# hpcaitech/SkyComputing

Hardware: AMD Instinct MI355X
Metric: sec_per_iter_bert160_mnli_bsz32 (lower is better)
Workload: dtype bf16; 1 GPU; model=bert-160L-H1024-A16, global_batch=32, seq_len=128, parallelism=pp1, microbatches=1, schedule=gpipe, allocate=even, num_pipeline_layers=483, hipgraph=True

## Files before the change

skycomputing_amd/ops/hip/attention.hip:

```cpp

#include "attn_common.h"

#define K_OFF 0
#define VT_OFF 0
#define P_OFF (16 * 1024)
#define ATT_LDS_BYTES (48 * 1024)

template <bool HAS_MASK, bool SAVE_ML, bool PROBS_MODE, bool TRV = false>
__global__ __launch_bounds__(256, 2) void attn_fwd_kernel(
    const ushort_t* __restrict__ qkv, const ushort_t* __restrict__ mask,
    ushort_t* __restrict__ out, float* __restrict__ m_io,
    float* __restrict__ l_io, ushort_t* __restrict__ p_out,
    ushort_t* __restrict__ pd_out, int B, int S, int h, float scale,
    float keep, uint64_t salt, const unsigned long long* __restrict__ state) {
  extern __shared__ __attribute__((aligned(16))) char lds[];
  const int tid = threadIdx.x;
  const int l = tid & 63;
  const int w = tid >> 6;
  const int bh = blockIdx.x;
  const int b = bh / h;
  const int hh = bh % h;
  const int ts = 3 * h * ATT_D;
  const int NT = (S + 15) / 16;
  const uint64_t seed = rng_seed(salt, state);
// ... 123 lines not shown
  att_zero(oacc[1]);

  __syncthreads();
  if (TRV) {
    att_glds_rows(vbase, ts, 0, 128, true, S, lds, VT_OFF, tid);
    asm volatile("s_waitcnt vmcnt(0)" ::: "memory");
  } else {
    if (S < ATT_SMAX) {
      for (int u = tid; u < (16 * 1024) / 16; u += 256)
        *(ushort8_t*)lds_at(lds, VT_OFF + u * 16) = (ushort8_t)(ushort_t)0;
      __syncthreads();
    }
    for (int u = tid; u < S * 8; u += 256) {
      const int tok = u >> 3;
      const int c16 = u & 7;
      ushort8_t v = *(const ushort8_t*)(vbase + (size_t)tok * ts + c16 * 8);
#pragma unroll
      for (int jj = 0; jj < 8; ++jj) {
        const int j = (jj + tok) & 7;
        const int c = c16 * 8 + j;
        *(ushort_t*)lds_at(lds, swz(VT_OFF + c * 256 + tok * 2, c, 15)) = v[j];
      }
    }
  }
  __syncthreads();

  for (int qi = 0; qi < 2; ++qi) {
    if ((qt0 + qi) * 16 >= S) break;
#pragma unroll
    for (int ks = 0; ks < 4; ++ks) {
      if (ks * 32 >= S) break;
      const int rl = qi * 16 + lm;
      bf16x8 ap = *(const bf16x8*)lds_at(
          lds, swz(P_OFF + w * 8192 + rl * 256 + (ks * 32 + lg * 8) * 2, rl, 15));
#pragma unroll
      for (int dvt = 0; dvt < 4; ++dvt) {
        bf16x8 bv;
        if (TRV) {
          bv = abf_tr_rows64(lds, VT_OFF, ks * 32 + lg * 8, dvt * 4, lm);
        } else {
          const int dv = dvt * 16 + lm;
          bv = *(const bf16x8*)lds_at(
              lds, swz(VT_OFF + dv * 256 + (ks * 32 + lg * 8) * 2, dv, 15));
        }
        oacc[qi][dvt] =
            __builtin_amdgcn_mfma_f32_16x16x32_bf16(ap, bv, oacc[qi][dvt], 0, 0, 0);
      }
    }
  }
  ushort_t* obase = out + ((size_t)b * S * h + hh) * ATT_D;
#pragma unroll
  for (int qi = 0; qi < 2; ++qi)
    att_store_rows16(obase, h * ATT_D, oacc[qi], (qt0 + qi) * 16, S, lm, lg);
}

template <int DT>
__global__ __launch_bounds__(256) void pack3_kernel(
    const void* __restrict__ s0, const void* __restrict__ s1,
    const void* __restrict__ s2, void* __restrict__ dst, int64_t B,
    int64_t S, int64_t h, int64_t d8) {
  const int64_t n = B * h * S * d8;
  for (int64_t u = (int64_t)blockIdx.x * 256 + threadIdx.x; u < n;
       u += (int64_t)gridDim.x * 256) {
    int64_t t = u;
    const int64_t di = t % d8; t /= d8;
    const int64_t tok = t % S; t /= S;
    const int64_t hh = t % h;
    const int64_t b = t / h;
    const int64_t src_off = u;
    const int64_t dst_base = (((b * S + tok) * 3) * h + hh) * d8 + di;
    float v[8];
    Vec8<DT>::load(s0, src_off, v);
    Vec8<DT>::store(dst, dst_base, v);
    Vec8<DT>::load(s1, src_off, v);
    Vec8<DT>::store(dst, dst_base + h * d8, v);
    Vec8<DT>::load(s2, src_off, v);
    Vec8<DT>::store(dst, dst_base + 2 * h * d8, v);
  }
}

SKY_EXPORT int sky_pack3(uint64_t stream, uint64_t s0, uint64_t s1,
                         uint64_t s2, uint64_t dst, int64_t B, int64_t S,
                         int64_t h, int64_t d, int dt) {
  if (d % 8 != 0) return (int)hipErrorInvalidValue;
  const int64_t n = B * h * S * (d / 8);
  unsigned grid = (unsigned)((n + 255) / 256);
  if (grid > 2048u) grid = 2048u;
  hipStream_t s = (hipStream_t)stream;
  if (dt == DT_F32)
    hipLaunchKernelGGL((pack3_kernel<DT_F32>), dim3(grid), dim3(256), 0, s,
                       (const void*)s0, (const void*)s1, (const void*)s2,
                       (void*)dst, B, S, h, d / 8);
  else
    hipLaunchKernelGGL((pack3_kernel<DT_BF16>), dim3(grid), dim3(256), 0, s,
                       (const void*)s0, (const void*)s1, (const void*)s2,
                       (void*)dst, B, S, h, d / 8);
  LAUNCH_CHECK();
  return 0;
}

static int attn_launch(uint64_t stream, uint64_t qkv, uint64_t mask,
                       uint64_t out, uint64_t m, uint64_t lsum, uint64_t p,
                       uint64_t pd, int64_t B, int64_t S, int64_t h,
                       int64_t d, float scale, float keep, uint64_t salt,
                       uint64_t state, bool probs_mode) {
  if (d != ATT_D || S > ATT_SMAX) return (int)hipErrorInvalidValue;
  hipStream_t s = (hipStream_t)stream;
  dim3 grid((unsigned)(B * h));
  size_t lds_bytes = ATT_LDS_BYTES;
  bool hm = mask != 0;
  const char* trve = getenv("SKY_ATTN_TRV");
  const bool trv = !(trve && trve[0] == '0');
#define ATT(SML, PM, TRV)                                                     \
  ATT_LAUNCH_HM(hm, (attn_fwd_kernel<HM, SML, PM, TRV>), grid, lds_bytes, s,  \
                (const ushort_t*)qkv, (const ushort_t*)mask, (ushort_t*)out,  \
                (float*)m, (float*)lsum, (ushort_t*)p, (ushort_t*)pd, (int)B, \
                (int)S, (int)h, scale, keep, salt,                            \
                (const unsigned long long*)state)
  if (probs_mode) { if (trv) ATT(false, true, true); else ATT(false, true, false); }
  else            { if (trv) ATT(true, false, true); else ATT(true, false, false); }
#undef ATT
  LAUNCH_CHECK();
  return 0;
}

SKY_EXPORT int sky_attn_fwd(uint64_t stream, uint64_t qkv, uint64_t mask,
                            uint64_t out, uint64_t m, uint64_t lsum,
                            int64_t B, int64_t S, int64_t h, int64_t d,
                            float scale, float keep, uint64_t salt,
                            uint64_t state) {
  return attn_launch(stream, qkv, mask, out, m, lsum, 0, 0, B, S, h, d,
                     scale, keep, salt, state, false);
}

SKY_EXPORT int sky_attn_probs(uint64_t stream, uint64_t qkv, uint64_t mask,
                              uint64_t m, uint64_t lsum, uint64_t p,
                              uint64_t pd, int64_t B, int64_t S, int64_t h,
                              int64_t d, float scale, float keep,
                              uint64_t salt, uint64_t state) {
  return attn_launch(stream, qkv, mask, 0, m, lsum, p, pd, B, S, h, d, scale,
                     keep, salt, state, true);
}
```

skycomputing_amd/ops/hip/attention_bwd.hip:

```cpp

#include "attn_common.h"

template <bool HAS_MASK, bool DBIAS>
__global__ __launch_bounds__(256, 3) void attn_bwd1s_kernel(
    const ushort_t* __restrict__ qkv, const ushort_t* __restrict__ dout,
    const ushort_t* __restrict__ mask, const float* __restrict__ m_io,
    const float* __restrict__ l_io, ushort_t* __restrict__ pdT,
    ushort_t* __restrict__ dsT, ushort_t* __restrict__ dqkv, int B, int S,
    int h, float scale, float keep, uint64_t salt,
    const unsigned long long* __restrict__ state, float* __restrict__ dbscr) {
  extern __shared__ __attribute__((aligned(16))) char lds[];
  const int tid = threadIdx.x;
  const int l = tid & 63;
  const int w = tid >> 6;
  const int lm = l & 15;
  const int lg = l >> 4;
  const int QB = (S + 63) / 64;
  const int bh = blockIdx.x / QB;
  const int qb = blockIdx.x % QB;
  const int b = bh / h;
  const int hh = bh % h;
  const int ts = 3 * h * ATT_D;
  const int NT = (S + 15) / 16;
  const uint64_t seed = rng_seed(salt, state);
// ... 389 lines not shown
      att_store_rows16(dq, ts, qacc, qtok_base, S, lm, lg);
    }

#pragma unroll
    for (int ks2 = 0; ks2 < 2; ++ks2) {
      const int q0t = ks2 * 32 + lg * 8;
      bf16x8 apd[2], ads[2];
#pragma unroll
      for (int ki = 0; ki < 2; ++ki) {
        const int kt = 2 * w + ki;
        apd[ki] = abf_tr_rows128(lds, ABF_PD, q0t, kt * 4, lm);
        ads[ki] = abf_tr_rows128(lds, ABF_DS, q0t, kt * 4, lm);
      }
#pragma unroll
      for (int ct = 0; ct < 4; ++ct) {
        bf16x8 bq = abf_tr_rows64(lds, ABF_Q, pass * 64 + q0t, ct * 4, lm);
        bf16x8 bdo = abf_tr_rows64(lds, ABF_DO, pass * 64 + q0t, ct * 4, lm);
#pragma unroll
        for (int ki = 0; ki < 2; ++ki) {
          vacc[ki][ct] = __builtin_amdgcn_mfma_f32_16x16x32_bf16(apd[ki], bdo, vacc[ki][ct], 0, 0, 0);
          kacc[ki][ct] = __builtin_amdgcn_mfma_f32_16x16x32_bf16(ads[ki], bq, kacc[ki][ct], 0, 0, 0);
        }
      }
    }
    __syncthreads();
  }

  ushort_t* dk = dqkv + (size_t)b * S * ts + (size_t)(h + hh) * ATT_D;
  ushort_t* dv = dqkv + (size_t)b * S * ts + (size_t)(2 * h + hh) * ATT_D;
#pragma unroll
  for (int ki = 0; ki < 2; ++ki)
    att_store_rows16x2(dk, dv, ts, kacc[ki], vacc[ki], (2 * w + ki) * 16, S,
                       lm, lg);
}

SKY_EXPORT int sky_attn_bwd_fused(uint64_t stream, uint64_t qkv,
                                  uint64_t dout, uint64_t mask, uint64_t m,
                                  uint64_t lsum, uint64_t dqkv, int64_t B,
                                  int64_t S, int64_t h, int64_t d,
                                  float scale, float keep, uint64_t salt,
                                  uint64_t state) {
  if (d != ATT_D || S > ATT_SMAX) return (int)hipErrorInvalidValue;
  hipStream_t s = (hipStream_t)stream;
  dim3 grid((unsigned)(B * h));
  ATT_LAUNCH_HM(mask != 0, (attn_bwd_fused_kernel<HM>), grid, ABF_LDS, s,
                (const ushort_t*)qkv, (const ushort_t*)dout,
                (const ushort_t*)mask, (const float*)m, (const float*)lsum,
                (ushort_t*)dqkv, (int)B, (int)S, (int)h, scale, keep, salt,
                (const unsigned long long*)state);
  LAUNCH_CHECK();
  return 0;
}

template <bool DBIAS>
static void launch_attn_bwd_pair(hipStream_t s, uint64_t qkv, uint64_t dout,
                                 uint64_t mask, uint64_t m, uint64_t lsum,
                                 uint64_t pdT, uint64_t dsT, uint64_t dqkv,
                                 int64_t B, int64_t S, int64_t h, float scale,
                                 float keep, uint64_t salt, uint64_t state,
                                 float* dbscr) {
  dim3 grid((unsigned)(B * h * ((S + 63) / 64)));
  ATT_LAUNCH_HM(mask != 0, (attn_bwd1s_kernel<HM, DBIAS>), grid, 48 * 1024, s,
                (const ushort_t*)qkv, (const ushort_t*)dout,
                (const ushort_t*)mask, (const float*)m, (const float*)lsum,
                (ushort_t*)pdT, (ushort_t*)dsT, (ushort_t*)dqkv, (int)B,
                (int)S, (int)h, scale, keep, salt,
                (const unsigned long long*)state, dbscr);
  hipLaunchKernelGGL(attn_bwd2_kernel<DBIAS>, dim3((unsigned)(B * h)),
                     dim3(256), (DBIAS ? 34 : 32) * 1024, s,
                     (const ushort_t*)qkv, (const ushort_t*)dout,
                     (const ushort_t*)pdT, (const ushort_t*)dsT,
                     (ushort_t*)dqkv, (int)B, (int)S, (int)h, dbscr);
}

SKY_EXPORT int sky_attn_bwd(uint64_t stream, uint64_t qkv, uint64_t dout,
                            uint64_t mask, uint64_t m, uint64_t lsum,
                            uint64_t pdT, uint64_t dsT, uint64_t dqkv,
                            int64_t B, int64_t S, int64_t h, int64_t d,
                            float scale, float keep, uint64_t salt,
                            uint64_t state) {
  if (d != ATT_D || S > ATT_SMAX) return (int)hipErrorInvalidValue;
  launch_attn_bwd_pair<false>((hipStream_t)stream, qkv, dout, mask, m, lsum,
                              pdT, dsT, dqkv, B, S, h, scale, keep, salt,
                              state, nullptr);
  LAUNCH_CHECK();
  return 0;
}

static int attn_bwd_dbias_impl(uint64_t stream, uint64_t qkv, uint64_t dout,
                               uint64_t mask, uint64_t m, uint64_t lsum,
                               uint64_t pdT, uint64_t dsT, uint64_t dqkv,
                               int64_t B, int64_t S, int64_t h, int64_t d,
                               float scale, float keep, uint64_t salt,
                               uint64_t state, uint64_t scratch,
                               uint64_t dbias, int dbias_dt,
                               SkyFinishJob* job) {
  if (d != ATT_D || S > ATT_SMAX || scratch == 0 || dbias == 0)
    return (int)hipErrorInvalidValue;
  hipStream_t s = (hipStream_t)stream;
  launch_attn_bwd_pair<true>(s, qkv, dout, mask, m, lsum, pdT, dsT, dqkv, B, S,
                             h, scale, keep, salt, state, (float*)scratch);
  const int64_t cols = 3 * h * ATT_D, nslabs = B * ((S + 63) / 64);
  if (job)
    sky_finish_job_set(job, scratch, dbias, 0, 0, nslabs, cols, 1, dbias_dt);
  else
    sky_launch_colsum_final(s, (const float*)scratch, (void*)dbias, cols,
                            nslabs, dbias_dt);
  LAUNCH_CHECK();
  return 0;
}

SKY_EXPORT int sky_attn_bwd_dbias(uint64_t stream, uint64_t qkv, uint64_t dout,
                                  uint64_t mask, uint64_t m, uint64_t lsum,
                                  uint64_t pdT, uint64_t dsT, uint64_t dqkv,
                                  int64_t B, int64_t S, int64_t h, int64_t d,
                                  float scale, float keep, uint64_t salt,
                                  uint64_t state, uint64_t scratch,
                                  uint64_t dbias, int dbias_dt) {
  return attn_bwd_dbias_impl(stream, qkv, dout, mask, m, lsum, pdT, dsT, dqkv,
                             B, S, h, d, scale, keep, salt, state, scratch,
                             dbias, dbias_dt, nullptr);
}

SKY_EXPORT int sky_attn_bwd_dbias_parts(
    uint64_t stream, uint64_t qkv, uint64_t dout, uint64_t mask, uint64_t m,
    uint64_t lsum, uint64_t pdT, uint64_t dsT, uint64_t dqkv, int64_t B,
    int64_t S, int64_t h, int64_t d, float scale, float keep, uint64_t salt,
    uint64_t state, uint64_t scratch, uint64_t dbias, int dbias_dt,
    uint64_t job) {
  if (job == 0) return (int)hipErrorInvalidValue;
  ((SkyFinishJob*)job)->nv = 0;
  return attn_bwd_dbias_impl(stream, qkv, dout, mask, m, lsum, pdT, dsT, dqkv,
                             B, S, h, d, scale, keep, salt, state, scratch,
                             dbias, dbias_dt, (SkyFinishJob*)job);
}
```

skycomputing_amd/ops/hip/attn_common.h:

```cpp
#pragma once

#include "common.h"

typedef const __attribute__((address_space(1))) unsigned int* att_gas;
typedef __attribute__((address_space(3))) unsigned int* att_las;

typedef __attribute__((ext_vector_type(8))) short bf16x8;
typedef __attribute__((ext_vector_type(4))) float f32x4;

#define ATT_SMAX 128
#define ATT_D 64

DEV void* lds_at(char* base, int byte) { return (void*)(base + byte); }

DEV int swz(int byte_addr, int row, int rmask) {
  return byte_addr ^ ((row & rmask) << 4);
}

typedef __attribute__((ext_vector_type(4))) short s16x4_a;
typedef __attribute__((address_space(3))) s16x4_a* abf_las4;

DEV bf16x8 abf_tr_rows64(const char* lds_base, int off, int r0, int cq0,
                         int s4) {
  s16x4_a v[2];
#pragma unroll
  for (int half = 0; half < 2; ++half) {
    const int row = r0 + half * 4 + (s4 >> 2);
    const int byte = (off + row * 128 + (cq0 + (s4 & 3)) * 8) ^ ((row & 7) << 4);
    v[half] = __builtin_amdgcn_ds_read_tr16_b64_v4i16(
        (abf_las4)(lds_base + byte));
  }
  return (bf16x8){v[0][0], v[0][1], v[0][2], v[0][3],
                  v[1][0], v[1][1], v[1][2], v[1][3]};
}

DEV bf16x8 abf_tr_rows128(const char* lds_base, int off, int r0, int cq0,
                          int s4) {
  s16x4_a v[2];
#pragma unroll
  for (int half = 0; half < 2; ++half) {
    const int row = r0 + half * 4 + (s4 >> 2);
    const int byte = (off + (row & 63) * 256 + (cq0 + (s4 & 3)) * 8) ^
                     ((row & 15) << 4);
    v[half] = __builtin_amdgcn_ds_read_tr16_b64_v4i16(
        (abf_las4)(lds_base + byte));
  }
  return (bf16x8){v[0][0], v[0][1], v[0][2], v[0][3],
                  v[1][0], v[1][1], v[1][2], v[1][3]};
}

template <int N> DEV void att_zero(f32x4 (&acc)[N]) {
#pragma unroll
  for (int i = 0; i < N; ++i) acc[i] = (f32x4){0.f, 0.f, 0.f, 0.f};
}

DEV void att_mask_cols(float (&mval)[8], bool has_mask,
                       const ushort_t* __restrict__ mask, int b, int S,
                       int lm, int col0) {
#pragma unroll
  for (int kt = 0; kt < 8; ++kt) {
    const int col = col0 + kt * 16 + lm;
    float mv = 0.f;
    if (has_mask && col < S) mv = bf16_to_f32(mask[(size_t)b * S + col]);
    mval[kt] = (col < S) ? mv : -3.0e38f;
  }
}
template <bool HAS_MASK>
DEV void att_mask_cols(float (&mval)[8], const ushort_t* __restrict__ mask,
                       int b, int S, int lm) {
  att_mask_cols(mval, HAS_MASK, mask, b, S, lm, 0);
}

DEV float row16_sum(float v) {
#pragma unroll
  for (int off = 8; off > 0; off >>= 1) v += __shfl_xor(v, off, 64);
  return v;
}
DEV float row16_max(float v) {
#pragma unroll
  for (int off = 8; off > 0; off >>= 1) v = fmaxf(v, __shfl_xor(v, off, 64));
  return v;
}

DEV void att_score_tile(f32x4 (&acc)[8], const bf16x8 (&a)[2], char* lds,
                        int off, int nt, int lm, int lg) {
#pragma unroll
  for (int kt = 0; kt < 8; ++kt) {
    if (kt >= nt) continue;
    const int ktok = kt * 16 + lm;
#pragma unroll
    for (int ks = 0; ks < 2; ++ks) {
      bf16x8 bk = *(const bf16x8*)lds_at(
          lds, swz(off + ktok * 128 + (ks * 32 + lg * 8) * 2, ktok, 7));
      acc[kt] = __builtin_amdgcn_mfma_f32_16x16x32_bf16(a[ks], bk, acc[kt], 0, 0, 0);
    }
  }
}

DEV void att_glds_rows(const ushort_t* src, int tstride, int tok0, int nrows,
                       bool clamp, int S, char* lds, int off, int tid) {
  for (int u = tid; u < nrows * 8; u += 256) {
    const int tok = u >> 3;
    int gtok = tok0 + tok;
    if (clamp && gtok >= S) gtok = S - 1;
    const int c16s = (u & 7) ^ (tok & 7);
    __builtin_amdgcn_global_load_lds(
        (att_gas)(src + (size_t)gtok * tstride + c16s * 8),
        (att_las)lds_at(lds, off + u * 16), 16, 0, 0);
  }
}

DEV float att_prob(float s, float scale, float mv, float m, float inv_l,
                   bool valid) {
  float p = __expf(s * scale + mv - m) * inv_l;
  if (!valid) p = 0.f;
  return p;
}

DEV void att_drop_hash(uint64_t (&z)[2], uint64_t seed, int bh, int S,
                       int row, int lm) {
  const uint64_t base = ((uint64_t)bh * S + row) * 16 + lm;
  z[0] = rng_hash(seed, base * 2);
  z[1] = rng_hash(seed, base * 2 + 1);
}
DEV bool att_drop_keep(const uint64_t (&z)[2], int kt, unsigned keep16) {
  const uint64_t zz = kt < 4 ? z[0] : z[1];
  return (unsigned)((zz >> (16 * (kt & 3))) & 0xFFFFu) < keep16;
}

DEV void att_store_rows16(ushort_t* __restrict__ dst, int rstride,
                          const f32x4 (&acc)[4], int row0, int S, int lm,
                          int lg) {
#pragma unroll
  for (int ct = 0; ct < 4; ++ct) {
#pragma unroll
    for (int r = 0; r < 4; r += 2) {
      const int row = row0 + lg * 4 + r;
      const unsigned int v2 = f32x2_to_bf16x2(acc[ct][r], acc[ct][r + 1]);
      if (row < S) dst[(size_t)row * rstride + ct * 16 + lm] = (ushort_t)v2;
      if (row + 1 < S)
        dst[(size_t)(row + 1) * rstride + ct * 16 + lm] = (ushort_t)(v2 >> 16);
    }
  }
}

DEV void att_store_rows16x2(ushort_t* __restrict__ d0,
                            ushort_t* __restrict__ d1, int rstride,
                            const f32x4 (&a0)[4], const f32x4 (&a1)[4],
                            int row0, int S, int lm, int lg) {
#pragma unroll
  for (int ct = 0; ct < 4; ++ct) {
#pragma unroll
    for (int r = 0; r < 4; r += 2) {
      const int row = row0 + lg * 4 + r;
      const int c = ct * 16 + lm;
      const unsigned int v0 = f32x2_to_bf16x2(a0[ct][r], a0[ct][r + 1]);
      const unsigned int v1 = f32x2_to_bf16x2(a1[ct][r], a1[ct][r + 1]);
      if (row < S) {
        d0[(size_t)row * rstride + c] = (ushort_t)v0;
        d1[(size_t)row * rstride + c] = (ushort_t)v1;
      }
      if (row + 1 < S) {
        d0[(size_t)(row + 1) * rstride + c] = (ushort_t)(v0 >> 16);
        d1[(size_t)(row + 1) * rstride + c] = (ushort_t)(v1 >> 16);
      }
    }
  }
}

DEV void att_colsum_rows16(float (&cs)[4], const f32x4 (&acc)[4], int row0,
                           int S, int lg) {
#pragma unroll
  for (int ct = 0; ct < 4; ++ct) {
#pragma unroll
    for (int r = 0; r < 4; ++r)
      if (row0 + lg * 4 + r < S) cs[ct] += bf16_to_f32(f32_to_bf16(acc[ct][r]));
  }
}

DEV void att_colsum_wave(float (&cs)[4]) {
#pragma unroll
  for (int ct = 0; ct < 4; ++ct) {
    cs[ct] += __shfl_xor(cs[ct], 16, 64);
    cs[ct] += __shfl_xor(cs[ct], 32, 64);
  }
}

#define ATT_LAUNCH_HM(has_mask, KERNEL, grid, lds_bytes, stream, ...)         \
  do {                                                                        \
    if (has_mask) {                                                           \
      constexpr bool HM = true;                                               \
      hipLaunchKernelGGL(KERNEL, grid, dim3(256), lds_bytes, stream,          \
                         __VA_ARGS__);                                        \
    } else {                                                                  \
      constexpr bool HM = false;                                              \
      hipLaunchKernelGGL(KERNEL, grid, dim3(256), lds_bytes, stream,          \
                         __VA_ARGS__);                                        \
    }                                                                         \
  } while (0)
```

skycomputing_amd/ops/hip/mfma_probe.hip:

```cpp

#include "common.h"

typedef __attribute__((ext_vector_type(8))) short bf16x8;
typedef __attribute__((ext_vector_type(4))) float f32x4;

__global__ __launch_bounds__(64) void mfma_probe_kernel(
    const ushort_t* __restrict__ A, const ushort_t* __restrict__ B,
    float* __restrict__ D) {
  const int l = threadIdx.x;
  bf16x8 a, b;
#pragma unroll
  for (int j = 0; j < 8; ++j) {
    int i = l % 16, k = 8 * (l / 16) + j;
    a[j] = (short)A[i * 32 + k];
    int n = l % 16;
    b[j] = (short)B[k * 16 + n];
  }
  f32x4 acc = {0.f, 0.f, 0.f, 0.f};
  acc = __builtin_amdgcn_mfma_f32_16x16x32_bf16(a, b, acc, 0, 0, 0);
#pragma unroll
  for (int r = 0; r < 4; ++r) {
    int i = 4 * (l / 16) + r, n = l % 16;
    D[i * 16 + n] = acc[r];
  }
}

SKY_EXPORT int sky_mfma_probe(uint64_t stream, uint64_t A, uint64_t B,
                              uint64_t D) {
  hipLaunchKernelGGL(mfma_probe_kernel, dim3(1), dim3(64), 0,
                     (hipStream_t)stream, (const ushort_t*)A,
                     (const ushort_t*)B, (float*)D);
  LAUNCH_CHECK();
  return 0;
}

typedef const __attribute__((address_space(1))) unsigned int* gp_u32;
typedef __attribute__((address_space(3))) unsigned int* lp_u32;

__global__ __launch_bounds__(256) void glds_probe_kernel(
    const ushort_t* __restrict__ src, ushort_t* __restrict__ dst, int mode) {
  __shared__ __attribute__((aligned(16))) char lbuf[4096];
  const int tid = threadIdx.x;
  const int w = tid >> 6;
  const ushort_t* g = src + tid * 8;
  if (mode == 0) {
    __builtin_amdgcn_global_load_lds((gp_u32)g, (lp_u32)(lbuf + tid * 16), 16, 0, 0);
  } else {
    __builtin_amdgcn_global_load_lds((gp_u32)g, (lp_u32)(lbuf + w * 64 * 16), 16, 0, 0);
  }
  asm volatile("s_waitcnt vmcnt(0)" ::: "memory");
  __syncthreads();
  *(ushort8_t*)(dst + tid * 8) = *(const ushort8_t*)(lbuf + tid * 16);
}

SKY_EXPORT int sky_glds_probe(uint64_t stream, uint64_t src, uint64_t dst,
                              int mode) {
  hipLaunchKernelGGL(glds_probe_kernel, dim3(1), dim3(256), 0,
                     (hipStream_t)stream, (const ushort_t*)src,
                     (ushort_t*)dst, mode);
  LAUNCH_CHECK();
  return 0;
}
```

skycomputing_amd/ops/hiplib.py:

```python

from __future__ import annotations

import ctypes
import os

_LIB = None
_LIB_PATH = os.path.join(os.path.dirname(os.path.abspath(__file__)), "hip", "libskyhip.so")
_TRIED = False

_SIGNATURES: dict[str, list] = {}

FINISH_MAX_JOBS = 4

u64 = ctypes.c_uint64
i64 = ctypes.c_int64
i32 = ctypes.c_int32
f32 = ctypes.c_float
f64 = ctypes.c_double


class FinishJob(ctypes.Structure):

    _fields_ = [
        ("scratch", u64), ("out", u64 * 3), ("nslabs", i64), ("cols", i64),
        ("nv", i32), ("dtout", i32),
    ]


def _register_signatures(lib):
    sigs = {
        "sky_layernorm_fwd": [u64, u64, u64, u64, u64, u64, u64, u64, i64, i64, f32, i32, f32, u64, u64],
        "sky_layernorm_bwd": [u64, u64, u64, u64, u64, u64, u64, u64, u64, u64, u64, i64, i64, i32, f32, u64, u64, u64],
        "sky_layernorm_bwd_xsum": [u64, u64, u64, u64, u64, u64, u64, u64, u64, u64, u64, i64, i64, i32, f32, u64, u64, u64, u64],
        "sky_layernorm_bwd_xsum_ok": [i64],
        "sky_bias_gelu_fwd": [u64, u64, u64, u64, i64, i64, i32],
        "sky_bias_gelu_bwd": [u64, u64, u64, u64, u64, u64, u64, i64, i64, i32],
        "sky_masked_softmax_fwd": [u64, u64, u64, u64, i64, i64, i64, i64, f32, f32, u64, i32],
        "sky_masked_softmax_bwd": [u64, u64, u64, u64, i64, i64, i64, i64, f32, f32, u64, i32],
        "sky_embedding_fwd": [u64] * 12 + [i64, i64, i64, f32, i32],
        "sky_embedding_bwd": [u64] * 16 + [i64, i64, i32],
        "sky_sgd_step": [u64, u64, i64, f32, f32, f32, i32, i32],
        "sky_adamw_tick": [u64, u64, f64, f64],
        "sky_gradnorm_partials": [u64, u64, i64, u64, i32],
        "sky_gradnorm_finish": [u64, u64, i64, u64, f32],
        "sky_adamw_step": [u64, u64, i64, u64, f64, f64, f32, f32, i32, i32],
        "sky_xent_fwd": [u64, u64, u64, u64, u64, u64, i64, i64, i64, i64, i32],
        "sky_xent_finish": [u64, u64, u64, u64, i64, i64, i64],
        "sky_xent_bwd": [u64, u64, u64, u64, u64, u64, u64, u64, i64, i64, i64, i64, i32],
        "sky_detect_mem": [u64, u64],
        "sky_dropout_fwd": [u64, u64, u64, i64, f32, u64, u64, i32],
        "sky_dropout_bwd": [u64, u64, u64, i64, f32, u64, u64, i32],
        "sky_rng_tick": [u64, u64],
        "sky_colsum": [u64, u64, u64, u64, i64, i64, i32, i32],
        "sky_hblt_wgrad_bgrad": [u64, u64, u64, u64, u64, i64, i64, i64, i32],
        "sky_hblt_wgrad": [u64, u64, u64, u64, i64, i64, i64, i32],
        "sky_hblt_linear_gelu_aux": [u64, u64, u64, u64, u64, u64, i64, i64, i64, i32, i32],
        "sky_mfma_probe": [u64, u64, u64, u64],
        "sky_glds_probe": [u64, u64, u64, i32],
        "sky_probe_bf16_round": [u64, u64],
        "sky_gemm": [u64, u64, u64, u64, u64, u64, i64, i64, i64, i64, i64, i64, i32, i32, i32, i32, i32],
        "sky_gemm2": [u64, u64, u64, u64, u64, u64, u64, i64, i64, i64, i64, i64, i64, i32, i32, i32, i32],
        "sky_pack3": [u64, u64, u64, u64, u64, i64, i64, i64, i64, i32],
        "sky_attn_fwd": [u64, u64, u64, u64, u64, u64, i64, i64, i64, i64, f32, f32, u64, u64],
        "sky_attn_probs": [u64, u64, u64, u64, u64, u64, u64, i64, i64, i64, i64, f32, f32, u64, u64],
        "sky_attn_flash_fwd": [u64, u64, u64, u64, u64, u64, i64, i64, i64, i64, f32, f32, u64, u64],
        "sky_attn_bwd": [u64] * 9 + [i64, i64, i64, i64, f32, f32, u64, u64],
        "sky_attn_bwd_dbias": [u64] * 9 + [i64, i64, i64, i64, f32, f32, u64, u64, u64, u64, i32],
        "sky_attn_bwd_dbias_parts": [u64] * 9 + [i64, i64, i64, i64, f32, f32, u64, u64, u64, u64, i32, u64],
        "sky_layernorm_bwd_parts": [u64, u64, u64, u64, u64, u64, u64, u64, u64, u64, u64, i64, i64, i32, f32, u64, u64, u64, u64, u64],
        "sky_bias_gelu_bwd_parts": [u64, u64, u64, u64, u64, u64, u64, i64, i64, i32, u64],
        "sky_colsum_finish": [u64, u64, i32],
        "sky_attn_bwd_fused": [u64] * 7 + [i64, i64, i64, i64, f32, f32, u64, u64],
    }
    for name, argtypes in sigs.items():
        if hasattr(lib, name):
            fn = getattr(lib, name)
            fn.argtypes = argtypes
            fn.restype = ctypes.c_int
    return sigs


def lib():
    global _LIB, _TRIED
    if _LIB is None and not _TRIED:
        _TRIED = True
        if os.path.isfile(_LIB_PATH):
            _LIB = ctypes.CDLL(_LIB_PATH)
            _register_signatures(_LIB)
    return _LIB


def available() -> bool:
    return lib() is not None


def require():
    l = lib()
    if l is None:
        raise RuntimeError(
            f"skycomputing_amd HIP kernel library not found at {_LIB_PATH}. "
            "Build it with `python -m skycomputing_amd.ops.build` (or __graft_entry__.build()). "
            "Running CUDA tensors through the eager fallback is disabled so GPU runs "
            "cannot silently lose the native path; set SKY_ALLOW_EAGER_GPU=1 to override."
        )
    return l


def check(rc: int, name: str):
    if rc != 0:
        raise RuntimeError(f"{name} failed with hipError_t={rc}")
# ... 5 lines not shown
```

Baseline: 0.09963 sec/iter.

## Add key-row attention kernels splitting forward and backward over query/key blocks

Adds new attention forward and backward kernels that transpose the MFMA orientation (keys as rows) and split each batch-head across multiple 64-token query or key blocks. Forward now launches B*h*(S/64) blocks instead of B*h. Backward splits into a dQ kernel that also emits row dot products and a separate dK/dV kernel with dropout bits precomputed in LDS. Both are enabled by default through an environment switch. The aim is more parallelism and occupancy (4 blocks per CU) on short sequences. The cost is that K/V or Q/dO are reloaded per block and the backward does two passes of score recomputation.

```diff
diff --git a/skycomputing_amd/ops/hip/attention.hip b/skycomputing_amd/ops/hip/attention.hip
--- a/skycomputing_amd/ops/hip/attention.hip
+++ b/skycomputing_amd/ops/hip/attention.hip
@@ -199,6 +199,121 @@
 #pragma unroll
   for (int qi = 0; qi < 2; ++qi)
     att_store_rows16(obase, h * ATT_D, oacc[qi], (qt0 + qi) * 16, S, lm, lg);
+}
+
+#define KR_K_OFF KR_IMG0_OFF
+#define KR_V_OFF KR_IMG1_OFF
+#define KR_MASK_OFF KR_AUX_OFF
+#define KR_LDS_BYTES (KR_AUX_OFF + 512)
+
+template <bool HAS_MASK, int QPW>
+__global__ __launch_bounds__(256, 4) void attn_fwd_krows_kernel(
+    const ushort_t* __restrict__ qkv, const ushort_t* __restrict__ mask,
+    ushort_t* __restrict__ out, float* __restrict__ m_io,
+    float* __restrict__ l_io, int B, int S, int h, float scale, float keep,
+    uint64_t salt, const unsigned long long* __restrict__ state) {
+  extern __shared__ __attribute__((aligned(16))) char lds[];
+  const int tid = threadIdx.x;
+  const int l = tid & 63;
+  const int w = tid >> 6;
+  const int lm = l & 15;
+  const int lg = l >> 4;
+  const int QB = (S + 64 * QPW - 1) / (64 * QPW);
+  const int bh = blockIdx.x / QB;
+  const int qb = blockIdx.x % QB;
+  const int b = bh / h;
+  const int hh = bh % h;
+  const int ts = 3 * h * ATT_D;
+  const int NT = (S + 15) / 16;
+  const int NP = (S + 31) / 32;
+  const uint64_t seed = rng_seed(salt, state);
+  const float inv_keep = 1.f / keep;
+  const unsigned keep16 = keep_to_16(keep);
+
+  const ushort_t* qbase = qkv + (size_t)b * S * ts + (size_t)hh * ATT_D;
+  const ushort_t* kbase = qbase + (size_t)h * ATT_D;
+  const ushort_t* vbase = qbase + (size_t)2 * h * ATT_D;
+  float* mk = (float*)lds_at(lds, KR_MASK_OFF);
+
+  att_glds_rows(kbase, ts, 0, NP * 32, true, S, lds, KR_K_OFF, tid);
+  att_glds_rows(vbase, ts, 0, NP * 32, true, S, lds, KR_V_OFF, tid);
+  att_mask_keys_lds(mk, HAS_MASK, mask, b, S, tid);
+  asm volatile("s_waitcnt vmcnt(0)" ::: "memory");
+  __syncthreads();
+
+  ushort_t* obase = out + ((size_t)b * S * h + hh) * ATT_D;
+#pragma clang loop unroll(disable)
+  for (int qi = 0; qi < QPW; ++qi) {
+    const int qtok_base = (qb * QPW + qi) * 64 + w * 16;
+    if (qtok_base >= S) break;
+    const int q = qtok_base + lm;
+    const int qc = q < S ? q : S - 1;
+    bf16x8 bq[2];
+#pragma unroll
+    for (int ks = 0; ks < 2; ++ks)
+      bq[ks] = *(const bf16x8*)(qbase + (size_t)qc * ts + ks * 32 + lg * 8);
+    f32x4 sacc[8];
+    att_zero(sacc);
+    att_score_tile_t(sacc, bq, lds, KR_K_OFF, NT, lm, lg);
+    float mx = -3.0e38f;
+#pragma unroll
+    for (int mt = 0; mt < 8; ++mt) {
+      if (mt >= NT) continue;
+      const f32x4 mv = att_mask_keys4(mk, mt, lg);
+#pragma unroll
+      for (int r = 0; r < 4; ++r) {
+        float zz = sacc[mt][r] * scale + mv[r];
+        sacc[mt][r] = zz;
+        mx = fmaxf(mx, zz);
+      }
+    }
+    mx = fmaxf(mx, __shfl_xor(mx, 16, 64));
+    mx = fmaxf(mx, __shfl_xor(mx, 32, 64));
+    float sm = 0.f;
+#pragma unroll
+    for (int mt = 0; mt < 8; ++mt) {
+      if (mt >= NT) continue;
+#pragma unroll
+      for (int r = 0; r < 4; ++r) {
+        float p = __expf(sacc[mt][r] - mx);
+        sacc[mt][r] = p;
+        sm += p;
+      }
+    }
+    sm += __shfl_xor(sm, 16, 64);
+    sm += __shfl_xor(sm, 32, 64);
+    const float inv = 1.f / sm;
+    if (lg == 0 && q < S) {
+      m_io[(size_t)bh * S + q] = mx;
+      l_io[(size_t)bh * S + q] = sm;
+    }
+    uint64_t z[4][2] = {{0, 0}, {0, 0}, {0, 0}, {0, 0}};
+    if (keep < 1.f) att_drop_hash_krows(z, seed, bh, S, q, lg);
+#pragma unroll
+    for (int mt = 0; mt < 8; ++mt) {
+      if (mt >= NT) continue;
+#pragma unroll
+      for (int r = 0; r < 4; ++r) {
+        float p = sacc[mt][r] * inv;
+        if (keep < 1.f) p = att_drop_keep(z[r], mt, keep16) ? p * inv_keep : 0.f;
+        sacc[mt][r] = p;
+      }
+    }
+    f32x4 oacc[4];
+    att_zero(oacc);
+#pragma unroll
+    for (int kp = 0; kp < 4; ++kp) {
+      if (kp >= NP) continue;
+      const bf16x8 bp = att_pack_dpair(sacc[2 * kp], sacc[2 * kp + 1]);
+#pragma unroll
+      for (int ct = 0; ct < 4; ++ct) {
+        const bf16x8 av = abf_tr_rows64_2(lds, KR_V_OFF, kp * 32 + lg * 4,
+                                          kp * 32 + 16 + lg * 4, ct * 4, lm);
+        oacc[ct] = __builtin_amdgcn_mfma_f32_16x16x32_bf16(av, bp, oacc[ct], 0, 0, 0);
+      }
+    }
+    att_store_cols16(obase, h * ATT_D, oacc, qtok_base, S, lm, lg);
+  }
 }
 
 template <int DT>
@@ -258,6 +373,21 @@
   bool hm = mask != 0;
   const char* trve = getenv("SKY_ATTN_TRV");
   const bool trv = !(trve && trve[0] == '0');
+  const char* kre = getenv("SKY_ATTN_KROWS");
+  if (!probs_mode && !(kre && kre[0] == '0')) {
+    const bool wide = kre && kre[0] == '2';
+    const int qspan = wide ? 128 : 64;
+    dim3 kgrid((unsigned)(B * h * ((S + qspan - 1) / qspan)));
+#define ATTK(QPW)                                                             \
+  ATT_LAUNCH_HM(hm, (attn_fwd_krows_kernel<HM, QPW>), kgrid, KR_LDS_BYTES, s, \
+                (const ushort_t*)qkv, (const ushort_t*)mask, (ushort_t*)out,  \
+                (float*)m, (float*)lsum, (int)B, (int)S, (int)h, scale, keep, \
+                salt, (const unsigned long long*)state)
+    if (wide) ATTK(2); else ATTK(1);
+#undef ATTK
+    LAUNCH_CHECK();
+    return 0;
+  }
 #define ATT(SML, PM, TRV)                                                     \
   ATT_LAUNCH_HM(hm, (attn_fwd_kernel<HM, SML, PM, TRV>), grid, lds_bytes, s,  \
                 (const ushort_t*)qkv, (const ushort_t*)mask, (ushort_t*)out,  \
diff --git a/skycomputing_amd/ops/hip/attention_bwd.hip b/skycomputing_amd/ops/hip/attention_bwd.hip
--- a/skycomputing_amd/ops/hip/attention_bwd.hip
+++ b/skycomputing_amd/ops/hip/attention_bwd.hip
@@ -465,6 +465,303 @@
   return 0;
 }
 
+#define KRB_K_OFF KR_IMG0_OFF
+#define KRB_V_OFF KR_IMG1_OFF
+#define KRB_MASK_OFF KR_AUX_OFF
+#define KRB_SUM_OFF (KR_AUX_OFF + 512)
+#define KRB_DQ_LDS (KR_AUX_OFF + 512 + 1024)
+
+template <bool HAS_MASK, bool DBIAS>
+__global__ __launch_bounds__(256, 4) void attn_bwd_dq_krows_kernel(
+    const ushort_t* __restrict__ qkv, const ushort_t* __restrict__ dout,
+    const ushort_t* __restrict__ mask, const float* __restrict__ m_io,
+    const float* __restrict__ l_io, float* __restrict__ dot_out,
+    ushort_t* __restrict__ dqkv, int B, int S, int h, float scale, float keep,
+    uint64_t salt, const unsigned long long* __restrict__ state,
+    float* __restrict__ dbscr) {
+  extern __shared__ __attribute__((aligned(16))) char lds[];
+  const int tid = threadIdx.x;
+  const int l = tid & 63;
+  const int w = tid >> 6;
+  const int lm = l & 15;
+  const int lg = l >> 4;
+  const int QB = (S + 63) / 64;
+  const int bh = blockIdx.x / QB;
+  const int qb = blockIdx.x % QB;
+  const int b = bh / h;
+  const int hh = bh % h;
+  const int ts = 3 * h * ATT_D;
+  const int dots = h * ATT_D;
+  const int NT = (S + 15) / 16;
+  const int NP = (S + 31) / 32;
+  const uint64_t seed = rng_seed(salt, state);
+  const float inv_keep = 1.f / keep;
+  const unsigned keep16 = keep_to_16(keep);
+
+  const ushort_t* qbase = qkv + (size_t)b * S * ts + (size_t)hh * ATT_D;
+  const ushort_t* kbase = qbase + (size_t)h * ATT_D;
+  const ushort_t* vbase = qbase + (size_t)2 * h * ATT_D;
+  const ushort_t* dobase = dout + ((size_t)b * S * h + hh) * ATT_D;
+  float* mk = (float*)lds_at(lds, KRB_MASK_OFF);
+
+  const int qtok_base = qb * 64 + w * 16;
+  const bool active = qtok_base < S;
+  const int q = qtok_base + lm;
+  const int qc = q < S ? q : S - 1;
+
+  att_glds_rows(kbase, ts, 0, NP * 32, true, S, lds, KRB_K_OFF, tid);
+  att_glds_rows(vbase, ts, 0, NP * 32, true, S, lds, KRB_V_OFF, tid);
+  att_mask_keys_lds(mk, HAS_MASK, mask, b, S, tid);
+  bf16x8 bq[2], bdo[2];
+#pragma unroll
+  for (int ks = 0; ks < 2; ++ks) {
+    bq[ks] = *(const bf16x8*)(qbase + (size_t)qc * ts + ks * 32 + lg * 8);
+    bdo[ks] = *(const bf16x8*)(dobase + (size_t)qc * dots + ks * 32 + lg * 8);
+  }
+  const float mrow = m_io[(size_t)bh * S + qc];
+  const float lrow = 1.f / l_io[(size_t)bh * S + qc];
+  asm volatile("s_waitcnt vmcnt(0)" ::: "memory");
+  __syncthreads();
+
+  float cs = 0.f;
+  if (active) {
+    f32x4 sacc[8], dacc[8];
+    att_zero(sacc);
+    att_zero(dacc);
+    att_score_tile_t(sacc, bq, lds, KRB_K_OFF, NT, lm, lg);
+    att_score_tile_t(dacc, bdo, lds, KRB_V_OFF, NT, lm, lg);
+    uint64_t z[4][2] = {{0, 0}, {0, 0}, {0, 0}, {0, 0}};
+    if (keep < 1.f) att_drop_hash_krows(z, seed, bh, S, q, lg);
+    float dot = 0.f;
+#pragma unroll
+    for (int mt = 0; mt < 8; ++mt) {
+      if (mt >= NT) continue;
+      const f32x4 mv = att_mask_keys4(mk, mt, lg);
+#pragma unroll
+      for (int r = 0; r < 4; ++r) {
+        const int key = mt * 16 + lg * 4 + r;
+        const float p = att_prob(sacc[mt][r], scale, mv[r], mrow, lrow,
+                                 q < S && key < S);
+        float dp = dacc[mt][r];
+        if (keep < 1.f)
+          dp = att_drop_keep(z[r], mt, keep16) ? dp * inv_keep : 0.f;
+        dot += dp * p;
+        sacc[mt][r] = p;
+        dacc[mt][r] = dp;
+      }
+    }
+    dot += __shfl_xor(dot, 16, 64);
+    dot += __shfl_xor(dot, 32, 64);
+    if (lg == 0 && q < S) dot_out[(size_t)bh * S + q] = dot;
+    f32x4 qacc[4];
+    att_zero(qacc);
+#pragma unroll
+    for (int kp = 0; kp < 4; ++kp) {
+      if (kp >= NP) continue;
+#pragma unroll
+      for (int t = 0; t < 2; ++t) {
+#pragma unroll
+        for (int r = 0; r < 4; ++r)
+          sacc[2 * kp + t][r] =
+              scale * sacc[2 * kp + t][r] * (dacc[2 * kp + t][r] - dot);
+      }
+      const bf16x8 bds = att_pack_dpair(sacc[2 * kp], sacc[2 * kp + 1]);
+#pragma unroll
+      for (int ct = 0; ct < 4; ++ct) {
+        const bf16x8 ak = abf_tr_rows64_2(lds, KRB_K_OFF, kp * 32 + lg * 4,
+                                          kp * 32 + 16 + lg * 4, ct * 4, lm);
+        qacc[ct] = __builtin_amdgcn_mfma_f32_16x16x32_bf16(ak, bds, qacc[ct], 0, 0, 0);
+      }
+    }
+    ushort_t* dq = dqkv + (size_t)b * S * ts + (size_t)hh * ATT_D;
+    att_store_cols16(dq, ts, qacc, qtok_base, S, lm, lg);
+    if constexpr (DBIAS) cs = att_colsum_cols16(qacc, qtok_base, S, lm);
+  }
+  if constexpr (DBIAS) {
+    float* wsum = (float*)lds_at(lds, KRB_SUM_OFF);
+    wsum[w * 64 + att_colsum_cols16_col(lm, lg)] = cs;
+    __syncthreads();
+    if (tid < 64)
+      dbscr[((size_t)b * QB + qb) * ts + (size_t)hh * ATT_D + tid] =
+          (wsum[tid] + wsum[64 + tid]) + (wsum[128 + tid] + wsum[192 + tid]);
+  }
+}
+
+#define KRB_Q_OFF KR_IMG0_OFF
+#define KRB_DO_OFF KR_IMG1_OFF
+#define KRB_STAT_OFF KR_AUX_OFF
+#define KRB_BITS_OFF (KR_AUX_OFF + 1536)
+#define KRB_SUM2_OFF (KR_AUX_OFF + 1536 + 2048)
+#define KRB_DKV_LDS (KR_AUX_OFF + 1536 + 2048 + 2048)
+
+template <bool HAS_MASK, bool DBIAS>
+__global__ __launch_bounds__(256, 4) void attn_bwd_dkv_krows_kernel(
+    const ushort_t* __restrict__ qkv, const ushort_t* __restrict__ dout,
+    const ushort_t* __restrict__ mask, const float* __restrict__ m_io,
+    const float* __restrict__ l_io, const float* __restrict__ dot_in,
+    ushort_t* __restrict__ dqkv, int B, int S, int h, float scale, float keep,
+    uint64_t salt, const unsigned long long* __restrict__ state,
+    float* __restrict__ dbscr) {
+  extern __shared__ __attribute__((aligned(16))) char lds[];
+  const int tid = threadIdx.x;
+  const int l = tid & 63;
+  const int w = tid >> 6;
+  const int lm = l & 15;
+  const int lg = l >> 4;
+  const int QB = (S + 63) / 64;
+  const int bh = blockIdx.x / QB;
+  const int kb = blockIdx.x % QB;
+  const int b = bh / h;
+  const int hh = bh % h;
+  const int ts = 3 * h * ATT_D;
+  const int dots = h * ATT_D;
+  const int NT = (S + 15) / 16;
+  const int NP = (S + 31) / 32;
+  const uint64_t seed = rng_seed(salt, state);
+  const float inv_keep = 1.f / keep;
+  const unsigned keep16 = keep_to_16(keep);
+
+  const ushort_t* qbase = qkv + (size_t)b * S * ts + (size_t)hh * ATT_D;
+  const ushort_t* kbase = qbase + (size_t)h * ATT_D;
+  const ushort_t* vbase = qbase + (size_t)2 * h * ATT_D;
+  const ushort_t* dobase = dout + ((size_t)b * S * h + hh) * ATT_D;
+  float* st = (float*)lds_at(lds, KRB_STAT_OFF);
+  unsigned char* bits = (unsigned char*)lds_at(lds, KRB_BITS_OFF);
+
+  const int ktok_base = kb * 64 + w * 16;
+  const bool active = ktok_base < S;
+  const int key = ktok_base + lm;
+  const int kc = key < S ? key : S - 1;
+
+  att_glds_rows(qbase, ts, 0, NP * 32, true, S, lds, KRB_Q_OFF, tid);
+  att_glds_rows(dobase, dots, 0, NP * 32, true, S, lds, KRB_DO_OFF, tid);
+  if (tid < ATT_SMAX) {
+    const bool live = tid < S;
+    st[tid] = live ? m_io[(size_t)bh * S + tid] : 0.f;
+    st[128 + tid] = live ? 1.f / l_io[(size_t)bh * S + tid] : 0.f;
+    st[256 + tid] = live ? dot_in[(size_t)bh * S + tid] : 0.f;
+  }
+  if (keep < 1.f)
+    att_drop_bits_lds(bits, seed, bh, S, kb, NP * 32, keep16, tid);
+  bf16x8 bk[2], bv[2];
+#pragma unroll
+  for (int ks = 0; ks < 2; ++ks) {
+    bk[ks] = *(const bf16x8*)(kbase + (size_t)kc * ts + ks * 32 + lg * 8);
+    bv[ks] = *(const bf16x8*)(vbase + (size_t)kc * ts + ks * 32 + lg * 8);
+  }
+  float mv = 0.f;
+  if (HAS_MASK && key < S) mv = bf16_to_f32(mask[(size_t)b * S + key]);
+  if (key >= S) mv = -3.0e38f;
+  asm volatile("s_waitcnt vmcnt(0)" ::: "memory");
+  __syncthreads();
+
+  float ck = 0.f, cv = 0.f;
+  if (active) {
+    f32x4 kacc[4], vacc[4];
+    att_zero(kacc);
+    att_zero(vacc);
+#pragma unroll
+    for (int qp = 0; qp < 4; ++qp) {
+      if (qp >= NP) continue;
+      f32x4 pd[2], ds[2];
+#pragma unroll
+      for (int t = 0; t < 2; ++t) {
+        const int qt = 2 * qp + t;
+        pd[t] = (f32x4){0.f, 0.f, 0.f, 0.f};
+        ds[t] = (f32x4){0.f, 0.f, 0.f, 0.f};
+        if (qt >= NT) continue;
+        const int qrow = qt * 16 + lm;
+        f32x4 s4 = {0.f, 0.f, 0.f, 0.f}, d4 = {0.f, 0.f, 0.f, 0.f};
+#pragma unroll
+        for (int ks = 0; ks < 2; ++ks) {
+          const bf16x8 aq = *(const bf16x8*)lds_at(
+              lds, swz(KRB_Q_OFF + qrow * 128 + (ks * 32 + lg * 8) * 2, qrow, 7));
+          const bf16x8 ado = *(const bf16x8*)lds_at(
+              lds, swz(KRB_DO_OFF + qrow * 128 + (ks * 32 + lg * 8) * 2, qrow, 7));
+          s4 = __builtin_amdgcn_mfma_f32_16x16x32_bf16(aq, bk[ks], s4, 0, 0, 0);
+          d4 = __builtin_amdgcn_mfma_f32_16x16x32_bf16(ado, bv[ks], d4, 0, 0, 0);
+        }
+        const f32x4 m4 = *(const f32x4*)(st + qt * 16 + lg * 4);
+        const f32x4 il4 = *(const f32x4*)(st + 128 + qt * 16 + lg * 4);
+        const f32x4 dot4 = *(const f32x4*)(st + 256 + qt * 16 + lg * 4);
+        unsigned kbits = 0xFFFFFFFFu;
+        if (keep < 1.f)
+          kbits = *(const unsigned*)(bits + ((qt * 4 + lg) * 16 + lm) * 4);
+#pragma unroll
+        for (int r = 0; r < 4; ++r) {
+          const int qq = qt * 16 + lg * 4 + r;
+          const float p = att_prob(s4[r], scale, mv, m4[r], il4[r],
+                                   qq < S && key < S);
+          const bool kbit = (kbits >> (8 * r + w)) & 1u;
+          float pdv = p, dp = d4[r];
+          if (keep < 1.f) {
+            pdv = kbit ? p * inv_keep : 0.f;
+            dp = kbit ? dp * inv_keep : 0.f;
+          }
+          pd[t][r] = pdv;
+          ds[t][r] = scale * p * (dp - dot4[r]);
+        }
+      }
+      const bf16x8 bpd = att_pack_dpair(pd[0], pd[1]);
+      const bf16x8 bds = att_pack_dpair(ds[0], ds[1]);
+#pragma unroll
+      for (int ct = 0; ct < 4; ++ct) {
+        const bf16x8 adot = abf_tr_rows64_2(lds, KRB_DO_OFF, qp * 32 + lg * 4,
+                                            qp * 32 + 16 + lg * 4, ct * 4, lm);
+        vacc[ct] = __builtin_amdgcn_mfma_f32_16x16x32_bf16(adot, bpd, vacc[ct], 0, 0, 0);
+        const bf16x8 aqt = abf_tr_rows64_2(lds, KRB_Q_OFF, qp * 32 + lg * 4,
+                                           qp * 32 + 16 + lg * 4, ct * 4, lm);
+        kacc[ct] = __builtin_amdgcn_mfma_f32_16x16x32_bf16(aqt, bds, kacc[ct], 0, 0, 0);
+      }
+    }
+    ushort_t* dk = dqkv + (size_t)b * S * ts + (size_t)(h + hh) * ATT_D;
+    ushort_t* dv = dqkv + (size_t)b * S * ts + (size_t)(2 * h + hh) * ATT_D;
+    att_store_cols16(dk, ts, kacc, ktok_base, S, lm, lg);
+    att_store_cols16(dv, ts, vacc, ktok_base, S, lm, lg);
+    if constexpr (DBIAS) {
+      ck = att_colsum_cols16(kacc, ktok_base, S, lm);
+      cv = att_colsum_cols16(vacc, ktok_base, S, lm);
+    }
+  }
+  if constexpr (DBIAS) {
+    float* wsum = (float*)lds_at(lds, KRB_SUM2_OFF);
+    const int c = att_colsum_cols16_col(lm, lg);
+    wsum[w * 128 + c] = ck;
+    wsum[w * 128 + 64 + c] = cv;
+    __syncthreads();
+    if (tid < 128) {
+      const size_t col = (size_t)((tid < 64 ? h : 2 * h) + hh) * ATT_D + (tid & 63);
+      dbscr[((size_t)b * QB + kb) * ts + col] =
+          (wsum[tid] + wsum[128 + tid]) + (wsum[256 + tid] + wsum[384 + tid]);
+    }
+  }
+}
+
+template <bool DBIAS>
+static void launch_attn_bwd_krows(hipStream_t s, uint64_t qkv, uint64_t dout,
+                                  uint64_t mask, uint64_t m, uint64_t lsum,
+                                  uint64_t pdT, uint64_t dqkv, int64_t B,
+                                  int64_t S, int64_t h, float scale,
+                                  float keep, uint64_t salt, uint64_t state,
+                                  float* dbscr) {
+  dim3 grid((unsigned)(B * h * ((S + 63) / 64)));
+  ATT_LAUNCH_HM(mask != 0, (attn_bwd_dq_krows_kernel<HM, DBIAS>), grid,
+                KRB_DQ_LDS, s, (const ushort_t*)qkv, (const ushort_t*)dout,
+                (const ushort_t*)mask, (const float*)m, (const float*)lsum,
+                (float*)pdT, (ushort_t*)dqkv, (int)B, (int)S, (int)h, scale,
+                keep, salt, (const unsigned long long*)state, dbscr);
+  ATT_LAUNCH_HM(mask != 0, (attn_bwd_dkv_krows_kernel<HM, DBIAS>), grid,
+                KRB_DKV_LDS, s, (const ushort_t*)qkv, (const ushort_t*)dout,
+                (const ushort_t*)mask, (const float*)m, (const float*)lsum,
+                (const float*)pdT, (ushort_t*)dqkv, (int)B, (int)S, (int)h,
+                scale, keep, salt, (const unsigned long long*)state, dbscr);
+}
+
+static bool attn_bwd_use_krows(int64_t S) {
+  const char* e = getenv("SKY_ATTN_KROWS");
+  return S >= 2 && !(e && e[0] == '0');
+}
+
 template <bool DBIAS>
 static void launch_attn_bwd_pair(hipStream_t s, uint64_t qkv, uint64_t dout,
                                  uint64_t mask, uint64_t m, uint64_t lsum,
@@ -493,9 +790,14 @@
                             float scale, float keep, uint64_t salt,
                             uint64_t state) {
   if (d != ATT_D || S > ATT_SMAX) return (int)hipErrorInvalidValue;
-  launch_attn_bwd_pair<false>((hipStream_t)stream, qkv, dout, mask, m, lsum,
-                              pdT, dsT, dqkv, B, S, h, scale, keep, salt,
-                              state, nullptr);
+  if (attn_bwd_use_krows(S))
+    launch_attn_bwd_krows<false>((hipStream_t)stream, qkv, dout, mask, m, lsum,
+                                 pdT, dqkv, B, S, h, scale, keep, salt, state,
+                                 nullptr);
+  else
+    launch_attn_bwd_pair<false>((hipStream_t)stream, qkv, dout, mask, m, lsum,
+                                pdT, dsT, dqkv, B, S, h, scale, keep, salt,
+                                state, nullptr);
   LAUNCH_CHECK();
   return 0;
 }
@@ -511,8 +813,12 @@
   if (d != ATT_D || S > ATT_SMAX || scratch == 0 || dbias == 0)
     return (int)hipErrorInvalidValue;
   hipStream_t s = (hipStream_t)stream;
-  launch_attn_bwd_pair<true>(s, qkv, dout, mask, m, lsum, pdT, dsT, dqkv, B, S,
-                             h, scale, keep, salt, state, (float*)scratch);
+  if (attn_bwd_use_krows(S))
+    launch_attn_bwd_krows<true>(s, qkv, dout, mask, m, lsum, pdT, dqkv, B, S, h,
+                                scale, keep, salt, state, (float*)scratch);
+  else
+    launch_attn_bwd_pair<true>(s, qkv, dout, mask, m, lsum, pdT, dsT, dqkv, B,
+                               S, h, scale, keep, salt, state, (float*)scratch);
   const int64_t cols = 3 * h * ATT_D, nslabs = B * ((S + 63) / 64);
   if (job)
     sky_finish_job_set(job, scratch, dbias, 0, 0, nslabs, cols, 1, dbias_dt);
diff --git a/skycomputing_amd/ops/hip/attn_common.h b/skycomputing_amd/ops/hip/attn_common.h
--- a/skycomputing_amd/ops/hip/attn_common.h
+++ b/skycomputing_amd/ops/hip/attn_common.h
@@ -10,6 +10,10 @@
 
 #define ATT_SMAX 128
 #define ATT_D 64
+
+#define KR_IMG0_OFF 0
+#define KR_IMG1_OFF (16 * 1024)
+#define KR_AUX_OFF (32 * 1024)
 
 DEV void* lds_at(char* base, int byte) { return (void*)(base + byte); }
 
@@ -32,6 +36,26 @@
   }
   return (bf16x8){v[0][0], v[0][1], v[0][2], v[0][3],
                   v[1][0], v[1][1], v[1][2], v[1][3]};
+}
+
+DEV bf16x8 abf_tr_rows64_2(const char* lds_base, int off, int ra, int rb,
+                           int cq0, int s4) {
+  s16x4_a v[2];
+#pragma unroll
+  for (int half = 0; half < 2; ++half) {
+    const int row = (half ? rb : ra) + (s4 >> 2);
+    const int byte = (off + row * 128 + (cq0 + (s4 & 3)) * 8) ^ ((row & 7) << 4);
+    v[half] = __builtin_amdgcn_ds_read_tr16_b64_v4i16(
+        (abf_las4)(lds_base + byte));
+  }
+  return (bf16x8){v[0][0], v[0][1], v[0][2], v[0][3],
+                  v[1][0], v[1][1], v[1][2], v[1][3]};
+}
+
+DEV bf16x8 att_pack_dpair(const f32x4& t0, const f32x4& t1) {
+  const uint4_t v = {f32x2_to_bf16x2(t0[0], t0[1]), f32x2_to_bf16x2(t0[2], t0[3]),
+                     f32x2_to_bf16x2(t1[0], t1[1]), f32x2_to_bf16x2(t1[2], t1[3])};
+  return __builtin_bit_cast(bf16x8, v);
 }
 
 DEV bf16x8 abf_tr_rows128(const char* lds_base, int off, int r0, int cq0,
@@ -95,6 +119,34 @@
       acc[kt] = __builtin_amdgcn_mfma_f32_16x16x32_bf16(a[ks], bk, acc[kt], 0, 0, 0);
     }
   }
+}
+
+DEV void att_score_tile_t(f32x4 (&acc)[8], const bf16x8 (&b)[2], char* lds,
+                          int off, int nt, int lm, int lg) {
+#pragma unroll
+  for (int mt = 0; mt < 8; ++mt) {
+    if (mt >= nt) continue;
+    const int tok = mt * 16 + lm;
+#pragma unroll
+    for (int ks = 0; ks < 2; ++ks) {
+      bf16x8 at = *(const bf16x8*)lds_at(
+          lds, swz(off + tok * 128 + (ks * 32 + lg * 8) * 2, tok, 7));
+      acc[mt] = __builtin_amdgcn_mfma_f32_16x16x32_bf16(at, b[ks], acc[mt], 0, 0, 0);
+    }
+  }
+}
+
+DEV void att_mask_keys_lds(float* mk, bool has_mask,
+                           const ushort_t* __restrict__ mask, int b, int S,
+                           int tid) {
+  if (tid < ATT_SMAX) {
+    float mv = 0.f;
+    if (has_mask && tid < S) mv = bf16_to_f32(mask[(size_t)b * S + tid]);
+    mk[tid] = (tid < S) ? mv : -3.0e38f;
+  }
+}
+DEV f32x4 att_mask_keys4(const float* mk, int mt, int lg) {
+  return *(const f32x4*)(mk + mt * 16 + lg * 4);
 }
 
 DEV void att_glds_rows(const ushort_t* src, int tstride, int tok0, int nrows,
@@ -117,15 +169,37 @@
   return p;
 }
 
+DEV uint64_t att_drop_hash_half(uint64_t seed, int bh, int S, int row, int lm,
+                                int half) {
+  const uint64_t base = ((uint64_t)bh * S + row) * 16 + lm;
+  return rng_hash(seed, base * 2 + half);
+}
 DEV void att_drop_hash(uint64_t (&z)[2], uint64_t seed, int bh, int S,
                        int row, int lm) {
-  const uint64_t base = ((uint64_t)bh * S + row) * 16 + lm;
-  z[0] = rng_hash(seed, base * 2);
-  z[1] = rng_hash(seed, base * 2 + 1);
+  z[0] = att_drop_hash_half(seed, bh, S, row, lm, 0);
+  z[1] = att_drop_hash_half(seed, bh, S, row, lm, 1);
 }
 DEV bool att_drop_keep(const uint64_t (&z)[2], int kt, unsigned keep16) {
   const uint64_t zz = kt < 4 ? z[0] : z[1];
   return (unsigned)((zz >> (16 * (kt & 3))) & 0xFFFFu) < keep16;
+}
+DEV void att_drop_hash_krows(uint64_t (&z)[4][2], uint64_t seed, int bh,
+                             int S, int q, int lg) {
+#pragma unroll
+  for (int r = 0; r < 4; ++r) att_drop_hash(z[r], seed, bh, S, q, lg * 4 + r);
+}
+DEV void att_drop_bits_lds(unsigned char* bits, uint64_t seed, int bh, int S,
+                           int kb, int nrows, unsigned keep16, int tid) {
+  for (int u = tid; u < nrows * 16; u += 256) {
+    const int q = u >> 4, lm = u & 15;
+    uint64_t z[2] = {0, 0};
+    z[kb & 1] = att_drop_hash_half(seed, bh, S, q, lm, kb & 1);
+    unsigned v = 0;
+#pragma unroll
+    for (int w = 0; w < 4; ++w)
+      v |= (unsigned)att_drop_keep(z, (kb & 1) * 4 + w, keep16) << w;
+    bits[(q >> 2) * 64 + lm * 4 + (q & 3)] = (unsigned char)v;
+  }
 }
 
 DEV void att_store_rows16(ushort_t* __restrict__ dst, int rstride,
@@ -186,6 +260,41 @@
   }
 }
 
+DEV void att_store_cols16(ushort_t* __restrict__ dst, int rstride,
+                          const f32x4 (&acc)[4], int row0, int S, int lm,
+                          int lg) {
+  const int row = row0 + lm;
+  if (row >= S) return;
+#pragma unroll
+  for (int ct = 0; ct < 4; ++ct)
+    *(ushort4_t*)(dst + (size_t)row * rstride + ct * 16 + lg * 4) =
+        f32x4_to_bf16x4(acc[ct][0], acc[ct][1], acc[ct][2], acc[ct][3]);
+}
+
+DEV float att_colsum_cols16(const f32x4 (&acc)[4], int row0, int S, int lm) {
+  const bool live = row0 + lm < S;
+  float v8[8], v4[4], v2[2];
+#pragma unroll
+  for (int i = 0; i < 8; ++i) {
+    const float lo = live ? bf16_to_f32(f32_to_bf16(acc[i >> 2][i & 3])) : 0.f;
+    const float hi =
+        live ? bf16_to_f32(f32_to_bf16(acc[2 + (i >> 2)][i & 3])) : 0.f;
+    v8[i] = ((lm & 8) ? hi : lo) + __shfl_xor((lm & 8) ? lo : hi, 8, 64);
+  }
+#pragma unroll
+  for (int i = 0; i < 4; ++i)
+    v4[i] = ((lm & 4) ? v8[4 + i] : v8[i]) +
+            __shfl_xor((lm & 4) ? v8[i] : v8[4 + i], 4, 64);
+#pragma unroll
+  for (int i = 0; i < 2; ++i)
+    v2[i] = ((lm & 2) ? v4[2 + i] : v4[i]) +
+            __shfl_xor((lm & 2) ? v4[i] : v4[2 + i], 2, 64);
+  return ((lm & 1) ? v2[1] : v2[0]) + __shfl_xor((lm & 1) ? v2[0] : v2[1], 1, 64);
+}
+DEV int att_colsum_cols16_col(int lm, int lg) {
+  return (lm >> 2) * 16 + lg * 4 + (lm & 3);
+}
+
 #define ATT_LAUNCH_HM(has_mask, KERNEL, grid, lds_bytes, stream, ...)         \
   do {                                                                        \
     if (has_mask) {                                                           \
diff --git a/skycomputing_amd/ops/hip/mfma_probe.hip b/skycomputing_amd/ops/hip/mfma_probe.hip
--- a/skycomputing_amd/ops/hip/mfma_probe.hip
+++ b/skycomputing_amd/ops/hip/mfma_probe.hip
@@ -1,8 +1,5 @@
 
-#include "common.h"
-
-typedef __attribute__((ext_vector_type(8))) short bf16x8;
-typedef __attribute__((ext_vector_type(4))) float f32x4;
+#include "attn_common.h"
 
 __global__ __launch_bounds__(64) void mfma_probe_kernel(
     const ushort_t* __restrict__ A, const ushort_t* __restrict__ B,
@@ -34,6 +31,47 @@
   return 0;
 }
 
+__global__ __launch_bounds__(64) void mfma_chain_probe_kernel(
+    const ushort_t* __restrict__ A, const ushort_t* __restrict__ B,
+    const ushort_t* __restrict__ A2, float* __restrict__ D2) {
+  __shared__ __attribute__((aligned(16))) char img[32 * 128];
+  const int l = threadIdx.x;
+  const int lm = l & 15, lg = l >> 4;
+  for (int u = l; u < 32 * 64; u += 64) {
+    const int k = u >> 6, i = u & 63;
+    *(ushort_t*)lds_at(img, swz(k * 128 + i * 2, k, 7)) =
+        i < 16 ? A2[i * 32 + k] : (ushort_t)0;
+  }
+  __syncthreads();
+  bf16x8 b;
+#pragma unroll
+  for (int j = 0; j < 8; ++j) b[j] = (short)B[(8 * lg + j) * 16 + lm];
+  f32x4 t[2];
+#pragma unroll
+  for (int tt = 0; tt < 2; ++tt) {
+    bf16x8 a;
+#pragma unroll
+    for (int j = 0; j < 8; ++j) a[j] = (short)A[(tt * 16 + lm) * 32 + 8 * lg + j];
+    t[tt] = (f32x4){0.f, 0.f, 0.f, 0.f};
+    t[tt] = __builtin_amdgcn_mfma_f32_16x16x32_bf16(a, b, t[tt], 0, 0, 0);
+  }
+  const bf16x8 bd = att_pack_dpair(t[0], t[1]);
+  const bf16x8 a2 = abf_tr_rows64_2(img, 0, lg * 4, 16 + lg * 4, 0, lm);
+  f32x4 acc = {0.f, 0.f, 0.f, 0.f};
+  acc = __builtin_amdgcn_mfma_f32_16x16x32_bf16(a2, bd, acc, 0, 0, 0);
+#pragma unroll
+  for (int r = 0; r < 4; ++r) D2[(4 * lg + r) * 16 + lm] = acc[r];
+}
+
+SKY_EXPORT int sky_mfma_chain_probe(uint64_t stream, uint64_t A, uint64_t B,
+                                    uint64_t A2, uint64_t D2) {
+  hipLaunchKernelGGL(mfma_chain_probe_kernel, dim3(1), dim3(64), 0,
+                     (hipStream_t)stream, (const ushort_t*)A,
+                     (const ushort_t*)B, (const ushort_t*)A2, (float*)D2);
+  LAUNCH_CHECK();
+  return 0;
+}
+
 typedef const __attribute__((address_space(1))) unsigned int* gp_u32;
 typedef __attribute__((address_space(3))) unsigned int* lp_u32;
 
diff --git a/skycomputing_amd/ops/hiplib.py b/skycomputing_amd/ops/hiplib.py
--- a/skycomputing_amd/ops/hiplib.py
+++ b/skycomputing_amd/ops/hiplib.py
@@ -56,6 +56,7 @@
         "sky_hblt_wgrad": [u64, u64, u64, u64, i64, i64, i64, i32],
         "sky_hblt_linear_gelu_aux": [u64, u64, u64, u64, u64, u64, i64, i64, i64, i32, i32],
         "sky_mfma_probe": [u64, u64, u64, u64],
+        "sky_mfma_chain_probe": [u64, u64, u64, u64, u64],
         "sky_glds_probe": [u64, u64, u64, i32],
         "sky_probe_bf16_round": [u64, u64],
         "sky_gemm": [u64, u64, u64, u64, u64, u64, i64, i64, i64, i64, i64, i64, i32, i32, i32, i32, i32],
```

Measured after the change: 0.09603 sec/iter (median of 6 runs). 1.04x faster.
